# sta105/VIORB

Measured on AMD Instinct MI355X. Metric: frames/sec ORB extract+match+pose-opt, EuRoC 752x480, 1/2/4/8 GPUs, higher is better.
Workload: dtype u8

## Files before the change

### viorb_amd/csrc/orb_extractor.hip

```cpp
#include <hip/hip_runtime.h>
#include <stdlib.h>
#include <math.h>
#include <vector>
#include <string>
#include <algorithm>
#include "viorb_common.h"
#include "orb_math.h"
#include "octree_arrays.h"

namespace viorb {

static const int8_t kPatternHost[1024] = {
#include "orb_pattern.inc"
};

enum { MINB = 16, PATCH = 31, HALF_PATCH = 15, MAX_LEVELS = 16 };

struct LevelDev {
    int w, h, stride;
    uint32_t plane_off;
    int cell_base, ncells;
    int quota;
    int oct_w, oct_h;
    int n_ini;
    float hx;
    float scale;
    float kp_size;
    int xtab_off, ytab_off;
    int kp_off;
    int oct_tier_cap;
};
struct CellDesc {
    int32_t level, x0, y0, cw, ch, shx, shy, pitch;
    uint32_t src_off;
    int32_t stride;
};

static inline int host_cv_round(double v) { return (int)nearbyint(v); }
static inline int host_cv_floor(double v) { int i = host_cv_round(v); float d = (float)(v - i); return i - (d < 0); }
static inline int host_cv_ceil(double v) { int i = host_cv_round(v); float d = (float)(i - v); return i + (d < 0); }
static inline int clampi(int v, int lo, int hi) { return v < lo ? lo : (v > hi ? hi : v); }
static inline size_t align_up(size_t v, size_t a) { return (v + a - 1) / a * a; }


struct XcdPlace { int nper, batch, xcd, img0; };
__device__ __forceinline__ bool xcd_place(const XcdPlace P, int& img, int& item) {
    const int L = blockIdx.x;
    if (P.xcd) { const int i = L >> 3, g = i / P.nper; item = i - g * P.nper; img = P.img0 + g * 8 + (L & 7); }
    else { img = L / P.nper; item = L - img * P.nper; img += P.img0; }
    return img < P.batch;
}
static inline XcdPlace make_place(int nper, int batch, int img0 = 0, int img1 = -1) {
    XcdPlace P; P.nper = nper; P.batch = img1 < 0 ? batch : std::min(batch, img1); P.xcd = batch >= 8; P.img0 = img0; return P;
}
static inline unsigned place_blocks(const XcdPlace& P) { const int n = P.batch - P.img0; return (unsigned)P.nper * (unsigned)(P.xcd ? 8 * ((n + 7) / 8) : n); }

__global__ void k_copy_level0(const uint8_t* __restrict__ src, int w, int h, int sstride, size_t spitch,
                              uint8_t* __restrict__ planes, size_t frame_bytes, int dstride, int* __restrict__ status, XcdPlace PL, int gx) {
    int b, item;
    if (!xcd_place(PL, b, item)) return;
    const int y = item / gx, bx = item - y * gx;
    if (item == 0 && threadIdx.x == 0) status[b] = 0;
    const int x = (bx * blockDim.x + threadIdx.x) * 16;
    if (x >= dstride) return;
    const uint8_t* s = src + (size_t)b * spitch + (size_t)y * sstride;
    uint8_t* d = planes + (size_t)b * frame_bytes + (size_t)y * dstride;
    uint32_t v[4];
    if (x + 16 <= w && ((((uintptr_t)(s + x)) & 15) == 0)) {
        const uint4 q = *reinterpret_cast<const uint4*>(s + x);
        v[0] = q.x; v[1] = q.y; v[2] = q.z; v[3] = q.w;
    } else {
#pragma unroll
        for (int k = 0; k < 4; k++) {
            uint32_t acc = 0;
#pragma unroll
            for (int j = 0; j < 4; j++) {
                int xx = x + 4 * k + j;
                uint32_t px = xx < w ? s[xx] : 0;
                acc |= px << (8 * j);
            }
            v[k] = acc;
        }
    }
    *reinterpret_cast<uint4*>(d + x) = make_uint4(v[0], v[1], v[2], v[3]);
}

#define RS_TW 64
#define RS_TH 16
__global__ __launch_bounds__(256) void k_resize(uint8_t* __restrict__ planes, size_t frame_bytes,
                                                const LevelDev* __restrict__ lv, int level,
                                                const int2* __restrict__ xtab_all,
                                                const int2* __restrict__ ytab_all, int lds_pitch_dw,
                                                int lds_rows, XcdPlace PL, int gx) {
    extern __shared__ uint32_t s_tile[];
    int b, item;
    if (!xcd_place(PL, b, item)) return;
    const int tby = item / gx, tbx = item - tby * gx;
    const LevelDev L = lv[level], P = lv[level - 1];
    const int2* xtab = xtab_all + L.xtab_off;
// ... 116 lines not shown
            packed |= (uint32_t)(val & 0xff) << (8 * j);
        }
        const int dxw = tx0 + xg * 4;
        if (dxw < A.dst_stride) *reinterpret_cast<uint32_t*>(dst + (size_t)dy * A.dst_stride + dxw) = packed;
    }
}

typedef unsigned short ushort2v __attribute__((ext_vector_type(2)));
__device__ __forceinline__ uint32_t dot2_u16(uint32_t a, uint32_t k, uint32_t c) {
    return __builtin_amdgcn_udot2(__builtin_bit_cast(ushort2v, a), __builtin_bit_cast(ushort2v, k), c, false);
}
#define RSS_LANES 32
#define RSS_PF 6
#define RSS_MAX_SRC_ROWS 60
struct ResizeStreamArgs {
    const uint8_t* planes; size_t frame_bytes;
    uint32_t src_off, dst_off;
    int src_stride, src_h, dst_stride, dst_w, dst_h;
    const int2* xtab; const int2* ytab; const uint2* etab; const int4* items;
};
struct __attribute__((packed, aligned(1))) rss_u8x8 { uint32_t lo, hi; };
__global__ __launch_bounds__(64) void k_resize_stream(ResizeStreamArgs A, XcdPlace PL) {
    int b, item;
    if (!xcd_place(PL, b, item)) return;
    const int4 t = A.items[item];
    const uint8_t* src = A.planes + (size_t)b * A.frame_bytes + A.src_off;
    uint8_t* dst = const_cast<uint8_t*>(A.planes) + (size_t)b * A.frame_bytes + A.dst_off;
    const int lane = threadIdx.x, hl = lane & (RSS_LANES - 1);
    const bool upper = lane >= RSS_LANES;
    const int Rb = t.z, y0A = t.y, y0B = t.y + Rb;
    const int rowsA = min(Rb, A.dst_h - y0A), rowsB = max(min(Rb, A.dst_h - y0B), 0);
    const int rsA = A.ytab[y0A].x & 0xffff, reA = A.ytab[y0A + rowsA - 1].x >> 16;
    const int rsB = rowsB > 0 ? A.ytab[min(y0B, A.dst_h - 1)].x & 0xffff : 0, reB = rowsB > 0 ? A.ytab[min(y0B + rowsB - 1, A.dst_h - 1)].x >> 16 : -1;
    const int ns = max(reA - rsA, reB - rsB) + 1;
    const int d = t.x + hl, sdw = A.dst_stride >> 2;
    uint32_t sel[4], aw[4]; int sxf = 0;
#pragma unroll
    for (int j = 0; j < 4; j++) {
        const int2 e = A.xtab[min(4 * d + j, A.dst_w - 1)];
        if (j == 0) sxf = e.x & 0xffff;
        sel[j] = (uint32_t)((e.x & 0xffff) - sxf) | ((uint32_t)((e.x >> 16) - sxf) << 16) | 0x0c000c00u;
        aw[j] = (uint32_t)e.y;
    }
    auto pack_entry = [&](int r0, int r1, int yb0, int nrows) {
        const int r = r0 + lane;
        const uint2 e = A.etab[min(r, A.src_h - 1)];
        const int y = (int)(e.x & 0x7fff) - yb0;
        const bool ok = r <= r1 && (e.x & 0x7fff) != 0x7fff && y >= 0 && y < nrows;
        return ok ? ((uint32_t)y | ((e.y & 0xfffu) << 7) | (((e.y >> 16) & 0xfffu) << 19) | ((e.x >> 15) << 31)) : 127u;
    };
    const uint32_t EA = pack_entry(rsA, reA, y0A, rowsA), EB = pack_entry(rsB, reB, y0B, rowsB);
    const uint8_t* pc = src + sxf;
    uint8_t* pd = dst + 4u * (uint32_t)min(d, sdw - 1);
    const bool col_ok = d < sdw;
    uint32_t lo[RSS_PF], hi[RSS_PF];
    auto request = [&](int i, uint32_t& l, uint32_t& h) {
        const uint32_t offA = __builtin_amdgcn_readfirstlane(min(rsA + i, A.src_h - 1) * A.src_stride), offB = __builtin_amdgcn_readfirstlane(min(rsB + i, A.src_h - 1) * A.src_stride);
        const rss_u8x8 v = *reinterpret_cast<const rss_u8x8*>(pc + (upper ? offB : offA));
        l = v.lo; h = v.hi;
    };
#pragma unroll
    for (int u = 0; u < RSS_PF; u++) request(u, lo[u], hi[u]);
    uint32_t hp[4] = {0, 0, 0, 0};
    for (int i0 = 0; i0 < ns; i0 += RSS_PF) {
#pragma unroll
        for (int u = 0; u < RSS_PF; u++) {
            const int i = i0 + u;
            uint32_t hc[4];
#pragma unroll
            for (int j = 0; j < 4; j++) {
                const uint32_t two = __builtin_amdgcn_perm(hi[u], lo[u], sel[j]);
                hc[j] = (dot2_u16(two, aw[j], 0u) & 0x7fff0u) << 5;
            }
            request(i + RSS_PF, lo[u], hi[u]);
            const uint32_t eA = __builtin_amdgcn_readlane(EA, i & 63), eB = __builtin_amdgcn_readlane(EB, i & 63);
            const uint32_t yrA = eA & 127u, yrB = eB & 127u;
            const bool emit = upper ? yrB < (uint32_t)rowsB : yrA < (uint32_t)rowsA;
            if (emit && col_ok) {
                const uint32_t b0 = upper ? (eB & (0xfffu << 7)) : (eA & (0xfffu << 7)), b1 = upper ? ((eB >> 12) & (0xfffu << 7)) : ((eA >> 12) & (0xfffu << 7));
                const uint32_t yoA = __builtin_amdgcn_readfirstlane((y0A + (int)yrA) * A.dst_stride), yoB = __builtin_amdgcn_readfirstlane((y0B + (int)yrB) * A.dst_stride);
                const uint32_t yo = upper ? yoB : yoA;
                uint32_t h0[4] = {hp[0], hp[1], hp[2], hp[3]};
                if ((int)(eA | eB) < 0) {
                    const bool same = upper ? (int)eB < 0 : (int)eA < 0;
#pragma unroll
                    for (int j = 0; j < 4; j++) h0[j] = same ? hc[j] : hp[j];
                }
                uint32_t v[4];
#pragma unroll
                for (int j = 0; j < 4; j++) {
                    const uint32_t t0 = (uint32_t)(((unsigned long long)h0[j] * b0) >> 32), t1 = (uint32_t)(((unsigned long long)hc[j] * b1) >> 32);
                    v[j] = (t0 + t1 + 2u) >> 2;
                }
                const uint32_t w01 = v[0] | (v[1] << 8), w23 = v[2] | (v[3] << 8);
// ... 649 lines not shown
template <class K> __device__ __forceinline__ void oct_sort(K* a, int m, int lane) {
    for (int k = 2; k <= m; k <<= 1)
        for (int j = k >> 1; j > 0; j >>= 1) {
            for (int t = lane; t < (m >> 1); t += 64) {
                const int lo = ((t & ~(j - 1)) << 1) | (t & (j - 1));
                const int hi = lo | j;
                const bool up = (lo & k) == 0;
                const K x = a[lo], y = a[hi];
                if ((x > y) == up) { a[lo] = y; a[hi] = x; }
            }
            WAVE_SYNC();
        }
}

template <bool BIG>
__global__ __launch_bounds__(64) void k_octree(const LevelDev* __restrict__ lv, const uint32_t* __restrict__ slots,
                                               int slot_cap, const int* __restrict__ cell_cnt, int ncells_total,
                                               uint32_t* __restrict__ lvl_kp, int kp_pitch, int* __restrict__ lvl_cnt,
                                               int* __restrict__ lvl_ncand, int nlevels, int* __restrict__ status,
                                               int ncap, int nodecap, int sortcap, int n_above, int n_upto,
                                               int level0, int use_tier_cap, int defer_nodes,
                                               uint32_t* __restrict__ big_scratch, int* __restrict__ big_next, int big_slots, int* __restrict__ lvl_tot,
                                               uint8_t* __restrict__ node_scratch = nullptr, size_t node_bytes = 0) {
    extern __shared__ __attribute__((aligned(16))) uint32_t s_oct[];
    typedef typename OctT<BIG>::Perm Perm; typedef typename OctT<BIG>::Node Node; typedef typename OctT<BIG>::SortKey SortKey;
    OctLdsT<BIG> S;
    if (BIG) {
        S.sortb = reinterpret_cast<SortKey*>(s_oct);
        S.nd = reinterpret_cast<Node*>(S.sortb + sortcap);
        S.keys = nullptr; S.perm0 = S.perm1 = nullptr;
    } else {
        S.keys = s_oct;
        S.perm0 = reinterpret_cast<Perm*>(s_oct + ncap);
        S.perm1 = S.perm0 + ncap;
        S.nd = reinterpret_cast<Node*>(S.perm1 + ncap);
        S.sortb = reinterpret_cast<SortKey*>(S.nd + nodecap);
    }
    const int lane = threadIdx.x, level = blockIdx.y + level0, b = blockIdx.x;
    const LevelDev L = lv[level];
// ... 210 lines not shown
            const Perm* pm = (o.flags & OCT_BUF) ? S.perm1 : S.perm0;
            uint32_t best = S.keys[pm[o.begin]];
            for (int k = 1; k < (int)o.count; k++) {
                const uint32_t key = S.keys[pm[o.begin + k]];
                if ((key >> 24) > (best >> 24)) best = key;
            }
            out[nn - 1 - i] = (best & 0xff000000u) | ((((best >> 12) & 0xfff) + MINB) << 12) | ((best & 0xfff) + MINB);
        }
    }
    if (lane == 0) {
        lvl_cnt[b * nlevels + level] = nn;
        if (overflow) status[b] = VIORB_ERR_CAPACITY;
    }
}

#define BS_LANES 32
#define BS_PF 6
__constant__ int c_gauss[7];
__global__ __launch_bounds__(64) void k_blur(const uint8_t* __restrict__ planes, uint8_t* __restrict__ blur,
                                             size_t frame_bytes, const LevelDev* __restrict__ lv,
                                             const int4* __restrict__ items, XcdPlace PL) {
    int b, item;
    if (!xcd_place(PL, b, item)) return;
    const int4 t = items[item];
    const LevelDev L = lv[t.x];
    const uint8_t* src = planes + (size_t)b * frame_bytes + L.plane_off;
    uint8_t* dst = blur + (size_t)b * frame_bytes + L.plane_off;
    const int lane = threadIdx.x, hl = lane & (BS_LANES - 1);
    const bool upper = lane >= BS_LANES;
    const int Rb = t.w, y0A = t.z, y0B = t.z + Rb;
// ... 358 lines not shown
    unsigned char* d_stereo_work = nullptr; size_t stereo_work_bytes = 0;
    bool oct_huge = false; uint8_t* d_oct_nodes = nullptr; size_t oct_node_bytes = 0;
    std::vector<int> rs_pitch_dw, rs_rows;
    std::vector<int4> rs2_tiles; std::vector<int> rs2_off, rs2_pitch_dw, rs2_ok; bool rs2_copy_ok = false;
    int4* d_rs2_tiles = nullptr;
    std::vector<int4> rss_items; std::vector<uint2> rss_etab; std::vector<int> rss_item_off, rss_etab_off, rss_ok;
    int4* d_rss_items = nullptr; uint2* d_rss_etab = nullptr;
    uint8_t *d_planes = nullptr, *d_blur = nullptr, *d_desc = nullptr, *d_stage = nullptr;
    LevelDev* d_lv = nullptr; CellDesc* d_cells = nullptr; int4* d_blur_tiles = nullptr;
    int2 *d_xtab = nullptr, *d_ytab = nullptr;
    uint32_t *d_slots = nullptr, *d_lvl_kp = nullptr;
    int *d_cell_cnt = nullptr, *d_lvl_cnt = nullptr, *d_lvl_ncand = nullptr, *d_count = nullptr, *d_status = nullptr;
    viorb_keypoint* d_kps = nullptr;
    size_t stage_bytes = 0;
    hipStream_t own_stream = nullptr;
    hipStream_t aux_stream = nullptr; hipEvent_t ev_fork = nullptr, ev_join = nullptr;
    hipStream_t last_stream = nullptr;
    int last_batch = 0;
    unsigned fast_prof_rot = 0;
    bool tables_uploaded = false;
};

static void free_device(viorb_extractor* h) {
    void* ptrs[] = {h->d_planes, h->d_blur, h->d_desc, h->d_stage, h->d_lv, h->d_cells, h->d_blur_tiles, h->d_xtab,
                    h->d_ytab, h->d_slots, h->d_lvl_kp, h->d_cell_cnt, h->d_lvl_cnt, h->d_lvl_ncand, h->d_count,
                    h->d_status, h->d_kps, h->d_rs2_tiles, h->d_rss_items, h->d_rss_etab, h->d_oct_big, h->d_oct_big_next, h->d_lvl_tot, h->d_oct_nodes};
    for (void* p : ptrs) if (p) (void)hipFree(p);
    h->d_rs2_tiles = nullptr; h->d_rss_items = nullptr; h->d_rss_etab = nullptr; h->d_oct_big = nullptr; h->d_oct_big_next = nullptr; h->d_lvl_tot = nullptr; h->d_oct_nodes = nullptr;
    h->d_planes = h->d_blur = h->d_desc = h->d_stage = nullptr; h->d_lv = nullptr; h->d_cells = nullptr;
    h->d_blur_tiles = nullptr; h->d_xtab = h->d_ytab = nullptr; h->d_slots = h->d_lvl_kp = nullptr;
    h->d_cell_cnt = h->d_lvl_cnt = h->d_lvl_ncand = h->d_count = h->d_status = nullptr; h->d_kps = nullptr;
// ... 62 lines not shown
                    max_cw = std::max(max_cw, (int)c.cw); max_ch = std::max(max_ch, (int)c.ch);
                }
            }
        }
        L.ncells = (int)h->cells.size() - L.cell_base;
        L.n_ini = (L.oct_h > 0 && L.oct_w > 0) ? (int)roundf((float)L.oct_w / (float)L.oct_h) : 0;
        L.hx = L.n_ini > 0 ? (float)L.oct_w / (float)L.n_ini : 1.f;
        L.kp_off = kp_off;
        kp_off += std::max(L.quota, 4 * L.n_ini) + 4;
        L.xtab_off = (int)xtab.size(); L.ytab_off = (int)ytab.size();
        if (l > 0) {
            const int sw = h->lv[l - 1].w, sh = h->lv[l - 1].h;
            const double inv_sx = (double)L.w / sw, inv_sy = (double)L.h / sh;
            const double scale_x = 1. / inv_sx, scale_y = 1. / inv_sy;
            for (int dx = 0; dx < L.w; dx++) {
                float fx = (float)((dx + 0.5) * scale_x - 0.5);
                int sx = host_cv_floor(fx);
                fx -= sx;
                if (sx < 0) { fx = 0; sx = 0; }
                if (sx + 1 >= sw && sx >= sw - 1) { fx = 0; sx = sw - 1; }
                const int a0 = clampi(host_cv_round((double)((1.f - fx) * 2048)), -32768, 32767);
                const int a1 = clampi(host_cv_round((double)(fx * 2048)), -32768, 32767);
                const int sx1 = std::min(sx + 1, sw - 1);
                xtab.push_back(make_int2(sx | (sx1 << 16), (a0 & 0xffff) | (a1 << 16)));
            }
            for (int dy = 0; dy < L.h; dy++) {
                float fy = (float)((dy + 0.5) * scale_y - 0.5);
                int sy = host_cv_floor(fy);
                fy -= sy;
                const int b0 = clampi(host_cv_round((double)((1.f - fy) * 2048)), -32768, 32767);
                const int b1 = clampi(host_cv_round((double)(fy * 2048)), -32768, 32767);
                const int sy0 = clampi(sy, 0, sh - 1), sy1 = clampi(sy + 1, 0, sh - 1);
                ytab.push_back(make_int2(sy0 | (sy1 << 16), (b0 & 0xffff) | (b1 << 16)));
            }
            int maxdw = 1, maxrows = 1;
            const int2* xt = xtab.data() + L.xtab_off; const int2* yt = ytab.data() + L.ytab_off;
            for (int tx = 0; tx < L.w; tx += RS_TW) {
                const int x1 = std::min(tx + RS_TW, L.w) - 1;
                const int xs0 = (xt[tx].x & 0xffff) & ~3, xs1 = xt[x1].x >> 16;
// ... 108 lines not shown
    size_t oct_lds = (size_t)h->oct_ncap * 8 + (size_t)h->oct_nodecap * sizeof(OctNode) + (size_t)sc * 4;
    if (h->oct_nodecap > 65535) { set_error("per-level quota %d too large for the quadtree's 16-bit node indices", maxq); return VIORB_ERR_UNSUPPORTED; }
    h->oct_huge = oct_lds > 160 * 1024;
    if (!h->oct_huge && oct_lds > 64 * 1024 &&
        raise_dynamic_lds(reinterpret_cast<const void*>(k_octree<false>), oct_lds) != hipSuccess) {
        (void)hipGetLastError();
        h->oct_ncap = 4096;
        oct_lds = (size_t)h->oct_ncap * 8 + (size_t)h->oct_nodecap * sizeof(OctNode) + (size_t)sc * 4;
        if (oct_lds > 64 * 1024) { set_error("quadtree LDS (%zu B) exceeds the dynamic-LDS limit", oct_lds); return VIORB_ERR_UNSUPPORTED; }
    }

    if (!h->oct_huge) {
        const size_t lds_big = (size_t)h->oct_sortcap * 8 + (size_t)h->oct_nodecap * sizeof(OctNodeBig);
        if (lds_big > 160 * 1024) h->oct_huge = true;
        else if (lds_big > 64 * 1024) VIORB_HIP_TRY(raise_dynamic_lds(reinterpret_cast<const void*>(k_octree<true>), lds_big));
    }
    {
        const char* e = getenv("VIORB_OCT_TIERS");
        std::string spec = e ? e : "3:2048";
        h->oct_tiers.clear();
        for (int l = 0; l < nl; l++) h->lv[l].oct_tier_cap = 0;
        int prev_l = 0, prev_c = std::min(h->oct_ncap, (int)OCT_NCAP_SMALL);
        h->oct_first_cap = prev_c;
        { const char* e2 = getenv("VIORB_OCT_NODE_X10"); h->oct_node_x10 = e2 ? atoi(e2) : 25; if (h->oct_node_x10 < 10 || h->oct_node_x10 > 50) h->oct_node_x10 = 50; }
        size_t pos = 0;
        while (!h->oct_huge && pos < spec.size()) {
            int l = 0, c = 0, used = 0;
            if (sscanf(spec.c_str() + pos, "%d:%d%n", &l, &c, &used) != 2) break;
            if (l == 0 && h->oct_tiers.empty() && c >= 64 && c <= prev_c) { h->oct_first_cap = c; prev_c = c + 1; }
            else if (l <= prev_l || l >= nl || c < 64 || c >= prev_c) break;
// ... 86 lines not shown
    }
    h->img_w = w; h->img_h = hgt;
    return VIORB_OK;
}

static int fast_launch_images(int batch) {
    static const int nlaunch = getenv("VIORB_FAST_LAUNCHES") ? std::max(1, atoi(getenv("VIORB_FAST_LAUNCHES"))) : FAST_LAUNCHES;
    return std::min(std::max(batch, 1), std::max(8, ((batch + nlaunch - 1) / nlaunch + 7) & ~7));
}

static int launch_all(viorb_extractor* h, const uint8_t* d_images, int batch, int stride, size_t pitch, hipStream_t st) {
    const int nl = h->p.nlevels;
    const int ncells = (int)h->cells.size();
    const LevelDev& L0 = h->lv[0];
    const bool fuse_copy = batch < 16 && nl > 1 && h->rs2_copy_ok && (stride & 3) == 0 && (pitch & 3) == 0 && (((uintptr_t)d_images) & 3) == 0 && (L0.w & 3) == 0;
    if (!fuse_copy) {
        const int gx = (L0.stride / 16 + 63) / 64;
        const XcdPlace PL = make_place(gx * L0.h, batch);
        ProfScope ps("k_copy_level0", st);
        hipLaunchKernelGGL(k_copy_level0, dim3(place_blocks(PL)), dim3(64), 0, st, d_images, L0.w, L0.h, stride, pitch, h->d_planes, h->frame_bytes, L0.stride, h->d_status, PL, gx);
    }
    for (int l = 1; l < nl; l++) {
        const LevelDev& L = h->lv[l];
        if (h->rss_ok[l] && !(l == 1 && fuse_copy)) {
            const LevelDev& P = h->lv[l - 1];
            ResizeStreamArgs A;
            A.planes = h->d_planes; A.frame_bytes = h->frame_bytes; A.src_off = P.plane_off; A.dst_off = L.plane_off;
            A.src_stride = P.stride; A.src_h = P.h; A.dst_stride = L.stride; A.dst_w = L.w; A.dst_h = L.h;
            A.xtab = h->d_xtab + L.xtab_off; A.ytab = h->d_ytab + L.ytab_off; A.etab = h->d_rss_etab + h->rss_etab_off[l];
            A.items = h->d_rss_items + h->rss_item_off[l];
            const int nitems = (l + 1 < nl ? h->rss_item_off[l + 1] : (int)h->rss_items.size()) - h->rss_item_off[l];
            const XcdPlace PL = make_place(nitems, batch);
            ProfScope ps("k_resize", st);
            hipLaunchKernelGGL(k_resize_stream, dim3(place_blocks(PL)), dim3(64), 0, st, A, PL);
            continue;
        }
        if (h->rs2_ok[l]) {
            const LevelDev& P = h->lv[l - 1];
            Resize2Args A;
            const bool from_image = (l == 1 && fuse_copy);
            A.src = from_image ? d_images : h->d_planes + P.plane_off; A.src_pitch = from_image ? pitch : h->frame_bytes; A.src_stride = from_image ? stride : P.stride;
            A.dst = h->d_planes + L.plane_off; A.dst_pitch = h->frame_bytes; A.dst_stride = L.stride; A.dst_w = L.w; A.dst_h = L.h;
            A.copy_dst = from_image ? h->d_planes + L0.plane_off : nullptr; A.copy_pitch = h->frame_bytes; A.copy_stride = L0.stride;
// ... 6 lines not shown
            hipLaunchKernelGGL(k_resize2, dim3(place_blocks(PL)), dim3(256), lds, st, A, PL);
            continue;
        }
        const int gx = (L.w + RS_TW - 1) / RS_TW, gy = (L.h + RS_TH - 1) / RS_TH;
        const XcdPlace PL = make_place(gx * gy, batch);
        const size_t lds = (size_t)h->rs_pitch_dw[l] * h->rs_rows[l] * 4;
        ProfScope ps("k_resize", st);
        hipLaunchKernelGGL(k_resize, dim3(place_blocks(PL)), dim3(256), lds, st, h->d_planes, h->frame_bytes, h->d_lv, l, h->d_xtab, h->d_ytab,
                           h->rs_pitch_dw[l], h->rs_rows[l], PL, gx);
    }
    {
        const size_t lds = h->fast_v3 ? (size_t)h->fast3_tile_bytes + h->fast3_score_bytes + (size_t)(F3_SURV_CAP + F3_CORN_CAP) * 2
                                      : (size_t)h->fast_tile_bytes + h->fast_score_bytes + (size_t)h->fast_list_cap * 4;
        const int step = fast_launch_images(batch);
        h->fast_prof_rot++;
        for (int i0 = 0; i0 < batch; i0 += step) {
            ProfScope ps(prof_times_everything() || (i0 / step) == (int)(h->fast_prof_rot % (unsigned)((batch + step - 1) / step)) ? "k_fast_cells" : nullptr, st);
            const XcdPlace PL = make_place((ncells + FAST_CELLS_PER_WAVE - 1) / FAST_CELLS_PER_WAVE, batch, i0, std::min(batch, i0 + step));
            if (h->fast_v3)
                hipLaunchKernelGGL(k_fast_cells3, dim3(place_blocks(PL)), dim3(64), lds, st, h->d_planes, h->frame_bytes, h->d_cells,
                                   h->p.ini_th_fast, h->p.min_th_fast, h->d_slots, h->slot_cap, h->d_cell_cnt, ncells, h->fast3_tile_bytes, h->fast3_score_bytes, PL);
            else
                hipLaunchKernelGGL(k_fast_cells, dim3(place_blocks(PL)), dim3(64), lds, st, h->d_planes, h->frame_bytes, h->d_lv, h->d_cells,
                                   h->p.ini_th_fast, h->p.min_th_fast, h->d_slots, h->slot_cap, h->d_cell_cnt, ncells,
                                   h->fast_tile_bytes, h->fast_score_bytes, h->fast_list_cap, PL);
        }
    }
    static const bool fork_blur = !(getenv("VIORB_BLUR_FORK") && atoi(getenv("VIORB_BLUR_FORK")) == 0);
    hipStream_t bst = st;
    if (fork_blur && batch >= 16) {
        if (!h->aux_stream) {
            VIORB_HIP_TRY(hipStreamCreateWithFlags(&h->aux_stream, hipStreamNonBlocking));
            VIORB_HIP_TRY(hipEventCreateWithFlags(&h->ev_fork, hipEventDisableTiming));
            VIORB_HIP_TRY(hipEventCreateWithFlags(&h->ev_join, hipEventDisableTiming));
        }
        bst = h->aux_stream;
        VIORB_HIP_TRY(hipEventRecord(h->ev_fork, st));
        VIORB_HIP_TRY(hipStreamWaitEvent(bst, h->ev_fork, 0));
    }
    {
        ProfScope ps("k_blur", bst);
        const XcdPlace PL = make_place((int)h->blur_tiles.size(), batch);
        hipLaunchKernelGGL(k_blur, dim3(place_blocks(PL)), dim3(64), 0, bst, h->d_planes, h->d_blur, h->frame_bytes,
                           h->d_lv, h->d_blur_tiles, PL);
    }
    if (bst != st) VIORB_HIP_TRY(hipEventRecord(h->ev_join, bst));
    {
        const size_t fixed = (size_t)h->oct_nodecap * sizeof(OctNode) + (size_t)h->oct_sortcap * 4;
        const int small = h->oct_first_cap > 0 ? h->oct_first_cap : std::min(h->oct_ncap, (int)OCT_NCAP_SMALL);
        const int ntier = h->oct_huge ? 0 : (int)h->oct_tiers.size();
        const bool defer = h->oct_node_x10 < 50;
        auto first_nodes = [&](int mq) { return std::min(5 * mq + 64, (h->oct_node_x10 * mq) / 10 + 64); };
        if (!h->oct_huge) {
            ProfScope ps("k_octree", st);
            const int l_end0 = ntier ? h->oct_tiers[0].first : nl;
            int mq0 = 1; for (int l = 0; l < l_end0; l++) mq0 = std::max(mq0, h->quota[l]);
            const int ndc0 = defer ? first_nodes(mq0) : h->oct_nodecap;
            hipLaunchKernelGGL(k_octree<false>, dim3(batch, l_end0), dim3(64), (size_t)small * 8 + (size_t)ndc0 * sizeof(OctNode) + (size_t)h->oct_sortcap * 4, st,
                               h->d_lv, h->d_slots, h->slot_cap, h->d_cell_cnt,
                               ncells, h->d_lvl_kp, h->kp_pitch, h->d_lvl_cnt, h->d_lvl_ncand, nl, h->d_status, small, ndc0,
                               h->oct_sortcap, -1, small, 0, 0, defer ? 1 : 0, nullptr, nullptr, 0, h->d_lvl_tot);
            for (int ti = 0; ti < ntier; ti++) {
                const int l0 = h->oct_tiers[ti].first, l1 = ti + 1 < ntier ? h->oct_tiers[ti + 1].first : nl, nc = h->oct_tiers[ti].second;
                int mq = 1; for (int l = l0; l < l1; l++) mq = std::max(mq, h->quota[l]);
                const int ndc = defer ? first_nodes(mq) : 5 * mq + 64;
                hipLaunchKernelGGL(k_octree<false>, dim3(batch, l1 - l0), dim3(64), (size_t)nc * 8 + (size_t)ndc * sizeof(OctNode) + (size_t)h->oct_sortcap * 4,
                                   st, h->d_lv, h->d_slots, h->slot_cap, h->d_cell_cnt, ncells, h->d_lvl_kp, h->kp_pitch, h->d_lvl_cnt, h->d_lvl_ncand, nl, h->d_status,
                                   nc, ndc, h->oct_sortcap, -1, nc, l0, 0, defer ? 1 : 0, nullptr, nullptr, 0, h->d_lvl_tot);
            }
        }
        if (!h->oct_huge && (small < h->oct_ncap || ntier || defer)) {
            ProfScope ps("k_octree_large", st);
            hipLaunchKernelGGL(k_octree<false>, dim3(batch, nl), dim3(64), (size_t)h->oct_ncap * 8 + fixed, st, h->d_lv, h->d_slots, h->slot_cap,
                               h->d_cell_cnt, ncells, h->d_lvl_kp, h->kp_pitch, h->d_lvl_cnt, h->d_lvl_ncand, nl, h->d_status, h->oct_ncap,
                               h->oct_nodecap, h->oct_sortcap, small, h->oct_ncap, 0, ntier ? 1 : 0, 0, nullptr, nullptr, 0, h->d_lvl_tot);
        }
        {
            const size_t lds_big = h->oct_huge ? 0 : (size_t)h->oct_sortcap * 8 + (size_t)h->oct_nodecap * sizeof(OctNodeBig);
            VIORB_HIP_TRY(hipMemsetAsync(h->d_oct_big_next, 0, sizeof(int), st));
            ProfScope ps("k_octree_big", st);
            hipLaunchKernelGGL(k_octree<true>, dim3(batch, nl), dim3(64), lds_big, st, h->d_lv, h->d_slots, h->slot_cap, h->d_cell_cnt, ncells, h->d_lvl_kp,
                               h->kp_pitch, h->d_lvl_cnt, h->d_lvl_ncand, nl, h->d_status, h->oct_big_cap, h->oct_nodecap, h->oct_sortcap,
                               h->oct_huge ? -1 : std::max(h->oct_ncap, (int)small), 0x7fffffff, 0, 0, 0, h->d_oct_big, h->d_oct_big_next, h->oct_big_slots, h->d_lvl_tot,
                               h->oct_huge ? h->d_oct_nodes : (uint8_t*)nullptr, h->oct_node_bytes);
        }
    }
    if (bst != st) VIORB_HIP_TRY(hipStreamWaitEvent(st, h->ev_join, 0));
    {
        ProfScope ps("k_orient_describe", st);
        const XcdPlace PL = make_place((h->out_cap + 3) / 4, batch);
        hipLaunchKernelGGL(k_orient_describe, dim3(place_blocks(PL)), dim3(256), 0, st, h->d_planes, h->d_blur, h->frame_bytes,
                           h->d_lv, nl, h->d_lvl_kp, h->kp_pitch, h->d_lvl_cnt, h->d_kps, h->d_desc, h->out_cap, h->d_count, h->d_status, PL);
    }
    VIORB_HIP_TRY(hipGetLastError());
    h->last_stream = st; h->last_batch = batch;
    return VIORB_OK;
}

extern "C" {
// ... 23 lines not shown
        for (v = 0; v <= vmax; ++v) h->umax[v] = host_cv_round(sqrt(hp2 - v * v));
        for (v = HALF_PATCH, v0 = 0; v >= vmin; --v) { while (h->umax[v0] == h->umax[v0 + 1]) ++v0; h->umax[v] = v0; ++v0; }
    }
    *out = h;
    return VIORB_OK;
}

int viorb_extractor_destroy(viorb_extractor* h) {
    if (!h) return VIORB_OK;
    if (h->d_planes) { (void)hipSetDevice(h->device); free_device(h); }
    if (h->d_stereo_work) (void)hipFree(h->d_stereo_work);
    if (h->own_stream) (void)hipStreamDestroy(h->own_stream);
    if (h->aux_stream) (void)hipStreamDestroy(h->aux_stream);
    if (h->ev_fork) (void)hipEventDestroy(h->ev_fork);
    if (h->ev_join) (void)hipEventDestroy(h->ev_join);
    delete h;
    return VIORB_OK;
}

int viorb_extractor_tables(const viorb_extractor* h, float* scale, float* inv_scale, float* sigma2, float* inv_sigma2,
                           int32_t* fpl) {
    VIORB_REQUIRE(h, "null handle");
    for (int i = 0; i < h->p.nlevels; i++) {
        if (scale) scale[i] = h->scale[i];
        if (inv_scale) inv_scale[i] = h->inv_scale[i];
        if (sigma2) sigma2[i] = h->sigma2[i];
        if (inv_sigma2) inv_sigma2[i] = h->inv_sigma2[i];
        if (fpl) fpl[i] = h->quota[i];
    }
    return VIORB_OK;
// ... 218 lines not shown
```

Baseline: 193,200.

## Fork level-0 copy onto side stream, band copy kernel, merge octree fallback launches

The level-0 copy kernel now handles an 8-row band per 64-lane block with prefetched 16-byte loads, and for large batches it runs on an auxiliary stream. Meanwhile level 1 is resized straight from the input images, so it no longer waits for the copy. The large and big octree fallback kernels are merged into one launch using a z-dimension role split, and the big_next counter reset moves into the small octree kernel in place of a memset. The resize window start is clamped so the 8-byte source read stays in bounds, and the weight shift is folded into the packed entry decode. These changes cut launch count and serialization, at the cost of extra stream and event management and shared-LDS sizing for the merged kernel.

Result: slower. 183,700 (-4.9%).

```diff
diff --git a/viorb_amd/csrc/orb_extractor.hip b/viorb_amd/csrc/orb_extractor.hip
--- a/viorb_amd/csrc/orb_extractor.hip
+++ b/viorb_amd/csrc/orb_extractor.hip
@@ -7,6 +7,7 @@
 #include "viorb_common.h"
 #include "orb_math.h"
 #include "octree_arrays.h"
+#include "resize_window.h"
 
 namespace viorb {
 
@@ -36,9 +37,6 @@
     int32_t stride;
 };
 
-static inline int host_cv_round(double v) { return (int)nearbyint(v); }
-static inline int host_cv_floor(double v) { int i = host_cv_round(v); float d = (float)(v - i); return i - (d < 0); }
-static inline int host_cv_ceil(double v) { int i = host_cv_round(v); float d = (float)(i - v); return i + (d < 0); }
 static inline int clampi(int v, int lo, int hi) { return v < lo ? lo : (v > hi ? hi : v); }
 static inline size_t align_up(size_t v, size_t a) { return (v + a - 1) / a * a; }
 
@@ -55,34 +53,59 @@
 }
 static inline unsigned place_blocks(const XcdPlace& P) { const int n = P.batch - P.img0; return (unsigned)P.nper * (unsigned)(P.xcd ? 8 * ((n + 7) / 8) : n); }
 
-__global__ void k_copy_level0(const uint8_t* __restrict__ src, int w, int h, int sstride, size_t spitch,
-                              uint8_t* __restrict__ planes, size_t frame_bytes, int dstride, int* __restrict__ status, XcdPlace PL, int gx) {
-    int b, item;
-    if (!xcd_place(PL, b, item)) return;
-    const int y = item / gx, bx = item - y * gx;
-    if (item == 0 && threadIdx.x == 0) status[b] = 0;
-    const int x = (bx * blockDim.x + threadIdx.x) * 16;
-    if (x >= dstride) return;
-    const uint8_t* s = src + (size_t)b * spitch + (size_t)y * sstride;
-    uint8_t* d = planes + (size_t)b * frame_bytes + (size_t)y * dstride;
-    uint32_t v[4];
-    if (x + 16 <= w && ((((uintptr_t)(s + x)) & 15) == 0)) {
-        const uint4 q = *reinterpret_cast<const uint4*>(s + x);
-        v[0] = q.x; v[1] = q.y; v[2] = q.z; v[3] = q.w;
-    } else {
-#pragma unroll
-        for (int k = 0; k < 4; k++) {
-            uint32_t acc = 0;
-#pragma unroll
-            for (int j = 0; j < 4; j++) {
-                int xx = x + 4 * k + j;
-                uint32_t px = xx < w ? s[xx] : 0;
-                acc |= px << (8 * j);
-            }
-            v[k] = acc;
-        }
-    }
-    *reinterpret_cast<uint4*>(d + x) = make_uint4(v[0], v[1], v[2], v[3]);
+#define CP_ROWS 8
+#define CP_PF 4
+__global__ __launch_bounds__(64) void k_copy_level0(const uint8_t* __restrict__ src, int w, int h, int sstride, size_t spitch,
+                                                    uint8_t* __restrict__ planes, size_t frame_bytes, int dstride, int* __restrict__ status, XcdPlace PL) {
+    int b, band;
+    if (!xcd_place(PL, b, band)) return;
+    const int lane = threadIdx.x;
+    if (band == 0 && lane == 0) status[b] = 0;
+    const int y0 = band * CP_ROWS, y1 = min(y0 + CP_ROWS, h);
+    const uint8_t* s = src + (size_t)b * spitch;
+    uint8_t* d = planes + (size_t)b * frame_bytes;
+    const bool aligned = (((uintptr_t)s | (uintptr_t)(uint32_t)sstride) & 15) == 0;
+    for (int x0 = 0; x0 < dstride; x0 += 64 * 16) {
+        const int x = x0 + lane * 16;
+        const bool wide = aligned && x + 16 <= w, bytes = !wide && x < w, pad = x >= w && x < dstride;
+        if (wide) {
+            for (int r0 = y0; r0 < y1; r0 += CP_PF) {
+                uint4 q[CP_PF];
+#pragma unroll
+                for (int u = 0; u < CP_PF; u++) {
+                    const uint32_t ro = __builtin_amdgcn_readfirstlane((uint32_t)(min(r0 + u, y1 - 1) * sstride));
+                    q[u] = *reinterpret_cast<const uint4*>(s + ro + (uint32_t)x);
+                }
+#pragma unroll
+                for (int u = 0; u < CP_PF; u++) {
+                    const uint32_t ro = __builtin_amdgcn_readfirstlane((uint32_t)(min(r0 + u, y1 - 1) * dstride));
+                    *reinterpret_cast<uint4*>(d + ro + (uint32_t)x) = q[u];
+                }
+            }
+        }
+        if (pad) {
+            for (int y = y0; y < y1; y++)
+                *reinterpret_cast<uint4*>(d + (uint32_t)__builtin_amdgcn_readfirstlane((uint32_t)(y * dstride)) + (uint32_t)x) = make_uint4(0u, 0u, 0u, 0u);
+        }
+        if (bytes) {
+            for (int y = y0; y < y1; y++) {
+                const uint8_t* sr = s + (size_t)(uint32_t)(y * sstride);
+                uint32_t v[4];
+#pragma unroll
+                for (int k = 0; k < 4; k++) {
+                    uint32_t acc = 0;
+#pragma unroll
+                    for (int j = 0; j < 4; j++) {
+                        const int xx = x + 4 * k + j;
+                        const uint32_t px = xx < w ? sr[xx] : 0;
+                        acc |= px << (8 * j);
+                    }
+                    v[k] = acc;
+                }
+                *reinterpret_cast<uint4*>(d + (size_t)(uint32_t)(y * dstride) + x) = make_uint4(v[0], v[1], v[2], v[3]);
+            }
+        }
+    }
 }
 
 #define RS_TW 64
@@ -229,9 +252,9 @@
 #define RSS_PF 6
 #define RSS_MAX_SRC_ROWS 60
 struct ResizeStreamArgs {
-    const uint8_t* planes; size_t frame_bytes;
-    uint32_t src_off, dst_off;
-    int src_stride, src_h, dst_stride, dst_w, dst_h;
+    const uint8_t* src; size_t src_pitch;
+    uint8_t* dst; size_t dst_pitch;
+    int src_stride, src_w, src_h, dst_stride, dst_w, dst_h;
     const int2* xtab; const int2* ytab; const uint2* etab; const int4* items;
 };
 struct __attribute__((packed, aligned(1))) rss_u8x8 { uint32_t lo, hi; };
@@ -239,8 +262,8 @@
     int b, item;
     if (!xcd_place(PL, b, item)) return;
     const int4 t = A.items[item];
-    const uint8_t* src = A.planes + (size_t)b * A.frame_bytes + A.src_off;
-    uint8_t* dst = const_cast<uint8_t*>(A.planes) + (size_t)b * A.frame_bytes + A.dst_off;
+    const uint8_t* src = A.src + (size_t)b * A.src_pitch;
+    uint8_t* dst = A.dst + (size_t)b * A.dst_pitch;
     const int lane = threadIdx.x, hl = lane & (RSS_LANES - 1);
     const bool upper = lane >= RSS_LANES;
     const int Rb = t.z, y0A = t.y, y0B = t.y + Rb;
@@ -249,14 +272,10 @@
     const int rsB = rowsB > 0 ? A.ytab[min(y0B, A.dst_h - 1)].x & 0xffff : 0, reB = rowsB > 0 ? A.ytab[min(y0B + rowsB - 1, A.dst_h - 1)].x >> 16 : -1;
     const int ns = max(reA - rsA, reB - rsB) + 1;
     const int d = t.x + hl, sdw = A.dst_stride >> 2;
-    uint32_t sel[4], aw[4]; int sxf = 0;
-#pragma unroll
-    for (int j = 0; j < 4; j++) {
-        const int2 e = A.xtab[min(4 * d + j, A.dst_w - 1)];
-        if (j == 0) sxf = e.x & 0xffff;
-        sel[j] = (uint32_t)((e.x & 0xffff) - sxf) | ((uint32_t)((e.x >> 16) - sxf) << 16) | 0x0c000c00u;
-        aw[j] = (uint32_t)e.y;
-    }
+    uint32_t sel[4], aw[4]; int2 xe[4];
+#pragma unroll
+    for (int j = 0; j < 4; j++) { xe[j] = A.xtab[min(4 * d + j, A.dst_w - 1)]; aw[j] = (uint32_t)xe[j].y; }
+    const int sxf = rss_window(xe, A.src_w, sel);
     auto pack_entry = [&](int r0, int r1, int yb0, int nrows) {
         const int r = r0 + lane;
         const uint2 e = A.etab[min(r, A.src_h - 1)];
@@ -285,14 +304,14 @@
 #pragma unroll
             for (int j = 0; j < 4; j++) {
                 const uint32_t two = __builtin_amdgcn_perm(hi[u], lo[u], sel[j]);
-                hc[j] = (dot2_u16(two, aw[j], 0u) & 0x7fff0u) << 5;
+                hc[j] = dot2_u16(two, aw[j], 0u) & 0x7fff0u;
             }
             request(i + RSS_PF, lo[u], hi[u]);
             const uint32_t eA = __builtin_amdgcn_readlane(EA, i & 63), eB = __builtin_amdgcn_readlane(EB, i & 63);
             const uint32_t yrA = eA & 127u, yrB = eB & 127u;
             const bool emit = upper ? yrB < (uint32_t)rowsB : yrA < (uint32_t)rowsA;
             if (emit && col_ok) {
-                const uint32_t b0 = upper ? (eB & (0xfffu << 7)) : (eA & (0xfffu << 7)), b1 = upper ? ((eB >> 12) & (0xfffu << 7)) : ((eA >> 12) & (0xfffu << 7));
+                const uint32_t b0 = upper ? ((eB << 5) & (0xfffu << 12)) : ((eA << 5) & (0xfffu << 12)), b1 = upper ? ((eB >> 7) & (0xfffu << 12)) : ((eA >> 7) & (0xfffu << 12));
                 const uint32_t yoA = __builtin_amdgcn_readfirstlane((y0A + (int)yrA) * A.dst_stride), yoB = __builtin_amdgcn_readfirstlane((y0B + (int)yrB) * A.dst_stride);
                 const uint32_t yo = upper ? yoB : yoA;
                 uint32_t h0[4] = {hp[0], hp[1], hp[2], hp[3]};
@@ -972,15 +991,16 @@
 }
 
 template <bool BIG>
-__global__ __launch_bounds__(64) void k_octree(const LevelDev* __restrict__ lv, const uint32_t* __restrict__ slots,
-                                               int slot_cap, const int* __restrict__ cell_cnt, int ncells_total,
-                                               uint32_t* __restrict__ lvl_kp, int kp_pitch, int* __restrict__ lvl_cnt,
-                                               int* __restrict__ lvl_ncand, int nlevels, int* __restrict__ status,
-                                               int ncap, int nodecap, int sortcap, int n_above, int n_upto,
-                                               int level0, int use_tier_cap, int defer_nodes,
-                                               uint32_t* __restrict__ big_scratch, int* __restrict__ big_next, int big_slots, int* __restrict__ lvl_tot,
-                                               uint8_t* __restrict__ node_scratch = nullptr, size_t node_bytes = 0) {
+__device__ __forceinline__ void octree_run(const LevelDev* __restrict__ lv, const uint32_t* __restrict__ slots,
+                                           int slot_cap, const int* __restrict__ cell_cnt, int ncells_total,
+                                           uint32_t* __restrict__ lvl_kp, int kp_pitch, int* __restrict__ lvl_cnt,
+                                           int* __restrict__ lvl_ncand, int nlevels, int* __restrict__ status,
+                                           int ncap, int nodecap, int sortcap, int n_above, int n_upto,
+                                           int level0, int use_tier_cap, int defer_nodes,
+                                           uint32_t* __restrict__ big_scratch, int* __restrict__ big_next, int big_slots, int* __restrict__ lvl_tot,
+                                           uint8_t* __restrict__ node_scratch = nullptr, size_t node_bytes = 0) {
     extern __shared__ __attribute__((aligned(16))) uint32_t s_oct[];
+    if (!BIG && big_next && blockIdx.x == 0 && blockIdx.y == 0 && threadIdx.x == 0) *big_next = 0;
     typedef typename OctT<BIG>::Perm Perm; typedef typename OctT<BIG>::Node Node; typedef typename OctT<BIG>::SortKey SortKey;
     OctLdsT<BIG> S;
     if (BIG) {
@@ -1221,6 +1241,34 @@
     }
 }
 
+template <bool BIG>
+__global__ __launch_bounds__(64) void k_octree(const LevelDev* __restrict__ lv, const uint32_t* __restrict__ slots,
+                                               int slot_cap, const int* __restrict__ cell_cnt, int ncells_total,
+                                               uint32_t* __restrict__ lvl_kp, int kp_pitch, int* __restrict__ lvl_cnt,
+                                               int* __restrict__ lvl_ncand, int nlevels, int* __restrict__ status,
+                                               int ncap, int nodecap, int sortcap, int n_above, int n_upto,
+                                               int level0, int use_tier_cap, int defer_nodes,
+                                               uint32_t* __restrict__ big_scratch, int* __restrict__ big_next, int big_slots, int* __restrict__ lvl_tot,
+                                               uint8_t* __restrict__ node_scratch = nullptr, size_t node_bytes = 0) {
+    octree_run<BIG>(lv, slots, slot_cap, cell_cnt, ncells_total, lvl_kp, kp_pitch, lvl_cnt, lvl_ncand, nlevels, status, ncap, nodecap, sortcap, n_above, n_upto,
+                    level0, use_tier_cap, defer_nodes, big_scratch, big_next, big_slots, lvl_tot, node_scratch, node_bytes);
+}
+
+struct OctRole { int ncap, nodecap, n_above, n_upto, use_tier_cap; };
+__global__ __launch_bounds__(64) void k_octree_fallback(const LevelDev* __restrict__ lv, const uint32_t* __restrict__ slots,
+                                                        int slot_cap, const int* __restrict__ cell_cnt, int ncells_total,
+                                                        uint32_t* __restrict__ lvl_kp, int kp_pitch, int* __restrict__ lvl_cnt,
+                                                        int* __restrict__ lvl_ncand, int nlevels, int* __restrict__ status, int sortcap,
+                                                        OctRole large, OctRole big, int first_role,
+                                                        uint32_t* __restrict__ big_scratch, int* __restrict__ big_next, int big_slots, int* __restrict__ lvl_tot) {
+    if (blockIdx.z + first_role == 0)
+        octree_run<false>(lv, slots, slot_cap, cell_cnt, ncells_total, lvl_kp, kp_pitch, lvl_cnt, lvl_ncand, nlevels, status, large.ncap, large.nodecap, sortcap,
+                          large.n_above, large.n_upto, 0, large.use_tier_cap, 0, nullptr, nullptr, 0, lvl_tot);
+    else
+        octree_run<true>(lv, slots, slot_cap, cell_cnt, ncells_total, lvl_kp, kp_pitch, lvl_cnt, lvl_ncand, nlevels, status, big.ncap, big.nodecap, sortcap,
+                         big.n_above, big.n_upto, 0, 0, 0, big_scratch, big_next, big_slots, lvl_tot);
+}
+
 #define BS_LANES 32
 #define BS_PF 6
 __constant__ int c_gauss[7];
@@ -1609,7 +1657,7 @@
     viorb_keypoint* d_kps = nullptr;
     size_t stage_bytes = 0;
     hipStream_t own_stream = nullptr;
-    hipStream_t aux_stream = nullptr; hipEvent_t ev_fork = nullptr, ev_join = nullptr;
+    hipStream_t aux_stream = nullptr; hipEvent_t ev_fork = nullptr, ev_join = nullptr, ev_copy = nullptr;
     hipStream_t last_stream = nullptr;
     int last_batch = 0;
     unsigned fast_prof_rot = 0;
@@ -1702,15 +1750,9 @@
             const double inv_sx = (double)L.w / sw, inv_sy = (double)L.h / sh;
             const double scale_x = 1. / inv_sx, scale_y = 1. / inv_sy;
             for (int dx = 0; dx < L.w; dx++) {
-                float fx = (float)((dx + 0.5) * scale_x - 0.5);
-                int sx = host_cv_floor(fx);
-                fx -= sx;
-                if (sx < 0) { fx = 0; sx = 0; }
-                if (sx + 1 >= sw && sx >= sw - 1) { fx = 0; sx = sw - 1; }
-                const int a0 = clampi(host_cv_round((double)((1.f - fx) * 2048)), -32768, 32767);
-                const int a1 = clampi(host_cv_round((double)(fx * 2048)), -32768, 32767);
-                const int sx1 = std::min(sx + 1, sw - 1);
-                xtab.push_back(make_int2(sx | (sx1 << 16), (a0 & 0xffff) | (a1 << 16)));
+                int pos, wts;
+                resize_x_entry(dx, sw, scale_x, pos, wts);
+                xtab.push_back(make_int2(pos, wts));
             }
             for (int dy = 0; dy < L.h; dy++) {
                 float fy = (float)((dy + 0.5) * scale_y - 0.5);
@@ -1849,6 +1891,8 @@
         const size_t lds_big = (size_t)h->oct_sortcap * 8 + (size_t)h->oct_nodecap * sizeof(OctNodeBig);
         if (lds_big > 160 * 1024) h->oct_huge = true;
         else if (lds_big > 64 * 1024) VIORB_HIP_TRY(raise_dynamic_lds(reinterpret_cast<const void*>(k_octree<true>), lds_big));
+        if (!h->oct_huge && std::max(oct_lds, lds_big) > 64 * 1024)
+            VIORB_HIP_TRY(raise_dynamic_lds(reinterpret_cast<const void*>(k_octree_fallback), std::max(oct_lds, lds_big)));
     }
     {
         const char* e = getenv("VIORB_OCT_TIERS");
@@ -1965,19 +2009,41 @@
     const int ncells = (int)h->cells.size();
     const LevelDev& L0 = h->lv[0];
     const bool fuse_copy = batch < 16 && nl > 1 && h->rs2_copy_ok && (stride & 3) == 0 && (pitch & 3) == 0 && (((uintptr_t)d_images) & 3) == 0 && (L0.w & 3) == 0;
+    auto side_stream = [&]() -> int {
+        if (!h->aux_stream) {
+            VIORB_HIP_TRY(hipStreamCreateWithFlags(&h->aux_stream, hipStreamNonBlocking));
+            VIORB_HIP_TRY(hipEventCreateWithFlags(&h->ev_fork, hipEventDisableTiming));
+            VIORB_HIP_TRY(hipEventCreateWithFlags(&h->ev_join, hipEventDisableTiming));
+            VIORB_HIP_TRY(hipEventCreateWithFlags(&h->ev_copy, hipEventDisableTiming));
+        }
+        return VIORB_OK;
+    };
+    static const bool fork_copy_env = !(getenv("VIORB_COPY_FORK") && atoi(getenv("VIORB_COPY_FORK")) == 0);
+    const bool fork_copy = fork_copy_env && !fuse_copy && batch >= 16 && nl > 1 && h->rss_ok[1];
     if (!fuse_copy) {
-        const int gx = (L0.stride / 16 + 63) / 64;
-        const XcdPlace PL = make_place(gx * L0.h, batch);
-        ProfScope ps("k_copy_level0", st);
-        hipLaunchKernelGGL(k_copy_level0, dim3(place_blocks(PL)), dim3(64), 0, st, d_images, L0.w, L0.h, stride, pitch, h->d_planes, h->frame_bytes, L0.stride, h->d_status, PL, gx);
+        hipStream_t cst = st;
+        if (fork_copy) {
+            if (side_stream() != VIORB_OK) return VIORB_ERR_HIP;
+            cst = h->aux_stream;
+            VIORB_HIP_TRY(hipEventRecord(h->ev_fork, st));
+            VIORB_HIP_TRY(hipStreamWaitEvent(cst, h->ev_fork, 0));
+        }
+        {
+            const XcdPlace PL = make_place((L0.h + CP_ROWS - 1) / CP_ROWS, batch);
+            ProfScope ps("k_copy_level0", cst);
+            hipLaunchKernelGGL(k_copy_level0, dim3(place_blocks(PL)), dim3(64), 0, cst, d_images, L0.w, L0.h, stride, pitch, h->d_planes, h->frame_bytes, L0.stride, h->d_status, PL);
+        }
+        if (fork_copy) VIORB_HIP_TRY(hipEventRecord(h->ev_copy, cst));
     }
     for (int l = 1; l < nl; l++) {
         const LevelDev& L = h->lv[l];
         if (h->rss_ok[l] && !(l == 1 && fuse_copy)) {
             const LevelDev& P = h->lv[l - 1];
             ResizeStreamArgs A;
-            A.planes = h->d_planes; A.frame_bytes = h->frame_bytes; A.src_off = P.plane_off; A.dst_off = L.plane_off;
-            A.src_stride = P.stride; A.src_h = P.h; A.dst_stride = L.stride; A.dst_w = L.w; A.dst_h = L.h;
+            const bool from_image = l == 1 && fork_copy;
+            A.src = from_image ? d_images : h->d_planes + P.plane_off; A.src_pitch = from_image ? pitch : h->frame_bytes; A.src_stride = from_image ? stride : P.stride;
+            A.dst = h->d_planes + L.plane_off; A.dst_pitch = h->frame_bytes;
+            A.src_w = P.w; A.src_h = P.h; A.dst_stride = L.stride; A.dst_w = L.w; A.dst_h = L.h;
             A.xtab = h->d_xtab + L.xtab_off; A.ytab = h->d_ytab + L.ytab_off; A.etab = h->d_rss_etab + h->rss_etab_off[l];
             A.items = h->d_rss_items + h->rss_item_off[l];
             const int nitems = (l + 1 < nl ? h->rss_item_off[l + 1] : (int)h->rss_items.size()) - h->rss_item_off[l];
@@ -2014,6 +2080,7 @@
                                       : (size_t)h->fast_tile_bytes + h->fast_score_bytes + (size_t)h->fast_list_cap * 4;
         const int step = fast_launch_images(batch);
         h->fast_prof_rot++;
+        if (fork_copy) VIORB_HIP_TRY(hipStreamWaitEvent(st, h->ev_copy, 0));
         for (int i0 = 0; i0 < batch; i0 += step) {
             ProfScope ps(prof_times_everything() || (i0 / step) == (int)(h->fast_prof_rot % (unsigned)((batch + step - 1) / step)) ? "k_fast_cells" : nullptr, st);
             const XcdPlace PL = make_place((ncells + FAST_CELLS_PER_WAVE - 1) / FAST_CELLS_PER_WAVE, batch, i0, std::min(batch, i0 + step));
@@ -2029,11 +2096,7 @@
     static const bool fork_blur = !(getenv("VIORB_BLUR_FORK") && atoi(getenv("VIORB_BLUR_FORK")) == 0);
     hipStream_t bst = st;
     if (fork_blur && batch >= 16) {
-        if (!h->aux_stream) {
-            VIORB_HIP_TRY(hipStreamCreateWithFlags(&h->aux_stream, hipStreamNonBlocking));
-            VIORB_HIP_TRY(hipEventCreateWithFlags(&h->ev_fork, hipEventDisableTiming));
-            VIORB_HIP_TRY(hipEventCreateWithFlags(&h->ev_join, hipEventDisableTiming));
-        }
+        if (side_stream() != VIORB_OK) return VIORB_ERR_HIP;
         bst = h->aux_stream;
         VIORB_HIP_TRY(hipEventRecord(h->ev_fork, st));
         VIORB_HIP_TRY(hipStreamWaitEvent(bst, h->ev_fork, 0));
@@ -2059,7 +2122,7 @@
             hipLaunchKernelGGL(k_octree<false>, dim3(batch, l_end0), dim3(64), (size_t)small * 8 + (size_t)ndc0 * sizeof(OctNode) + (size_t)h->oct_sortcap * 4, st,
                                h->d_lv, h->d_slots, h->slot_cap, h->d_cell_cnt,
                                ncells, h->d_lvl_kp, h->kp_pitch, h->d_lvl_cnt, h->d_lvl_ncand, nl, h->d_status, small, ndc0,
-                               h->oct_sortcap, -1, small, 0, 0, defer ? 1 : 0, nullptr, nullptr, 0, h->d_lvl_tot);
+                               h->oct_sortcap, -1, small, 0, 0, defer ? 1 : 0, nullptr, h->d_oct_big_next, 0, h->d_lvl_tot);
             for (int ti = 0; ti < ntier; ti++) {
                 const int l0 = h->oct_tiers[ti].first, l1 = ti + 1 < ntier ? h->oct_tiers[ti + 1].first : nl, nc = h->oct_tiers[ti].second;
                 int mq = 1; for (int l = l0; l < l1; l++) mq = std::max(mq, h->quota[l]);
@@ -2069,20 +2132,22 @@
                                    nc, ndc, h->oct_sortcap, -1, nc, l0, 0, defer ? 1 : 0, nullptr, nullptr, 0, h->d_lvl_tot);
             }
         }
-        if (!h->oct_huge && (small < h->oct_ncap || ntier || defer)) {
+        if (!h->oct_huge) {
+            const bool with_large = small < h->oct_ncap || ntier || defer;
+            const size_t lds_large = (size_t)h->oct_ncap * 8 + fixed, lds_big = (size_t)h->oct_sortcap * 8 + (size_t)h->oct_nodecap * sizeof(OctNodeBig);
+            OctRole RL, RB;
+            RL.ncap = h->oct_ncap; RL.nodecap = h->oct_nodecap; RL.n_above = small; RL.n_upto = h->oct_ncap; RL.use_tier_cap = ntier ? 1 : 0;
+            RB.ncap = h->oct_big_cap; RB.nodecap = h->oct_nodecap; RB.n_above = std::max(h->oct_ncap, (int)small); RB.n_upto = 0x7fffffff; RB.use_tier_cap = 0;
             ProfScope ps("k_octree_large", st);
-            hipLaunchKernelGGL(k_octree<false>, dim3(batch, nl), dim3(64), (size_t)h->oct_ncap * 8 + fixed, st, h->d_lv, h->d_slots, h->slot_cap,
-                               h->d_cell_cnt, ncells, h->d_lvl_kp, h->kp_pitch, h->d_lvl_cnt, h->d_lvl_ncand, nl, h->d_status, h->oct_ncap,
-                               h->oct_nodecap, h->oct_sortcap, small, h->oct_ncap, 0, ntier ? 1 : 0, 0, nullptr, nullptr, 0, h->d_lvl_tot);
-        }
-        {
-            const size_t lds_big = h->oct_huge ? 0 : (size_t)h->oct_sortcap * 8 + (size_t)h->oct_nodecap * sizeof(OctNodeBig);
+            hipLaunchKernelGGL(k_octree_fallback, dim3(batch, nl, with_large ? 2 : 1), dim3(64), with_large ? std::max(lds_large, lds_big) : lds_big, st,
+                               h->d_lv, h->d_slots, h->slot_cap, h->d_cell_cnt, ncells, h->d_lvl_kp, h->kp_pitch, h->d_lvl_cnt, h->d_lvl_ncand, nl, h->d_status,
+                               h->oct_sortcap, RL, RB, with_large ? 0 : 1, h->d_oct_big, h->d_oct_big_next, h->oct_big_slots, h->d_lvl_tot);
+        } else {
             VIORB_HIP_TRY(hipMemsetAsync(h->d_oct_big_next, 0, sizeof(int), st));
             ProfScope ps("k_octree_big", st);
-            hipLaunchKernelGGL(k_octree<true>, dim3(batch, nl), dim3(64), lds_big, st, h->d_lv, h->d_slots, h->slot_cap, h->d_cell_cnt, ncells, h->d_lvl_kp,
+            hipLaunchKernelGGL(k_octree<true>, dim3(batch, nl), dim3(64), 0, st, h->d_lv, h->d_slots, h->slot_cap, h->d_cell_cnt, ncells, h->d_lvl_kp,
                                h->kp_pitch, h->d_lvl_cnt, h->d_lvl_ncand, nl, h->d_status, h->oct_big_cap, h->oct_nodecap, h->oct_sortcap,
-                               h->oct_huge ? -1 : std::max(h->oct_ncap, (int)small), 0x7fffffff, 0, 0, 0, h->d_oct_big, h->d_oct_big_next, h->oct_big_slots, h->d_lvl_tot,
-                               h->oct_huge ? h->d_oct_nodes : (uint8_t*)nullptr, h->oct_node_bytes);
+                               -1, 0x7fffffff, 0, 0, 0, h->d_oct_big, h->d_oct_big_next, h->oct_big_slots, h->d_lvl_tot, h->d_oct_nodes, h->oct_node_bytes);
         }
     }
     if (bst != st) VIORB_HIP_TRY(hipStreamWaitEvent(st, h->ev_join, 0));
@@ -2136,6 +2201,7 @@
     if (h->aux_stream) (void)hipStreamDestroy(h->aux_stream);
     if (h->ev_fork) (void)hipEventDestroy(h->ev_fork);
     if (h->ev_join) (void)hipEventDestroy(h->ev_join);
+    if (h->ev_copy) (void)hipEventDestroy(h->ev_copy);
     delete h;
     return VIORB_OK;
 }
diff --git a/viorb_amd/csrc/resize_window.h b/viorb_amd/csrc/resize_window.h
--- /dev/null
+++ b/viorb_amd/csrc/resize_window.h
@@ -0,0 +1,35 @@
+#pragma once
+#include <math.h>
+#include <stdint.h>
+
+#if defined(__HIPCC__)
+#define RSW_HD __host__ __device__ inline
+#else
+#define RSW_HD inline
+#endif
+
+static inline int host_cv_round(double v) { return (int)nearbyint(v); }
+static inline int host_cv_floor(double v) { int i = host_cv_round(v); float d = (float)(v - i); return i - (d < 0); }
+static inline int host_cv_ceil(double v) { int i = host_cv_round(v); float d = (float)(i - v); return i + (d < 0); }
+
+static inline void resize_x_entry(int dx, int sw, double scale_x, int& pos, int& wts) {
+    float fx = (float)((dx + 0.5) * scale_x - 0.5);
+    int sx = host_cv_floor(fx);
+    fx -= sx;
+    if (sx < 0) { fx = 0; sx = 0; }
+    if (sx + 1 >= sw && sx >= sw - 1) { fx = 0; sx = sw - 1; }
+    int a0 = host_cv_round((double)((1.f - fx) * 2048)), a1 = host_cv_round((double)(fx * 2048));
+    a0 = a0 < -32768 ? -32768 : (a0 > 32767 ? 32767 : a0);
+    a1 = a1 < -32768 ? -32768 : (a1 > 32767 ? 32767 : a1);
+    const int sx1 = sx + 1 < sw - 1 ? sx + 1 : sw - 1;
+    pos = sx | (sx1 << 16);
+    wts = (a0 & 0xffff) | (a1 << 16);
+}
+
+template <class E> RSW_HD int rss_window(const E e[4], int src_w, uint32_t sel[4]) {
+    const int first = e[0].x & 0xffff;
+    const int start = src_w >= 8 ? (first < src_w - 8 ? first : src_w - 8) : first;
+    for (int j = 0; j < 4; j++)
+        sel[j] = (uint32_t)((e[j].x & 0xffff) - start) | ((uint32_t)((e[j].x >> 16) - start) << 16) | 0x0c000c00u;
+    return start;
+}
```
